# sahaRatul/sela

Hardware: NVIDIA H100
Metric: encode+decode MSamples/s (higher is better)
Workload: dtype f64+int64

## Files before the change

include/sela_b200.h:

```cpp
#ifndef SELA_B200_H_
#define SELA_B200_H_

#include <stddef.h>
#include <stdint.h>

#ifdef __cplusplus
extern "C" {
#endif

#define SELAB200_ABI_VERSION     2
#define SELAB200_FRAME_SAMPLES   2048
#define SELAB200_MAX_LPC_ORDER   100
#define SELAB200_MAX_RICE_PARAM  20
#define SELAB200_MAX_CHANNELS    16

typedef enum selab200_status {
    SELAB200_OK              = 0,
    SELAB200_ERR_NO_DEVICE   = -1,
    SELAB200_ERR_CUDA        = -2,
    SELAB200_ERR_ARGUMENT    = -3,
    SELAB200_ERR_CAPACITY    = -4,
    SELAB200_ERR_RANGE       = -5,
    SELAB200_ERR_BITSTREAM   = -6,
    SELAB200_ERR_NOT_INIT    = -7
// ... 65 lines not shown
    uint32_t header_frames;
    uint32_t n_frames;
    uint64_t n_words;
    uint64_t n_bytes_used;
} selab200_container_info;

size_t selab200_container_bound(uint32_t n_frames, uint32_t channels);

int selab200_encode_container(const int16_t *pcm, uint32_t n_frames, uint32_t channels,
                              uint32_t sample_rate, uint16_t bits_per_sample,
                              uint8_t *container, size_t capacity, size_t *bytes_used);

int selab200_container_info_get(const uint8_t *container, size_t n_bytes, selab200_container_info *info);

int selab200_container_frame_offsets(const uint8_t *container, size_t n_bytes, uint64_t *offsets,
                                     size_t capacity, selab200_container_info *info);

typedef struct selab200_container selab200_container;
int  selab200_container_open(const uint8_t *container, size_t n_bytes, selab200_container **handle,
                             selab200_container_info *info);
int  selab200_container_decode(selab200_container *handle, int16_t *pcm_out);
void selab200_container_close(selab200_container *handle);


int selab200_lpc_residues(const int32_t *samples, uint32_t n_sub, uint8_t *order,
                          int32_t *q, int32_t *residues);

int selab200_lpc_samples(const int32_t *residues, uint32_t n_sub, const uint8_t *order,
                         const int32_t *q, int32_t *samples);

int selab200_rice_encode(const int32_t *values, const uint32_t *counts, uint32_t n_streams,
                         uint32_t stride, uint32_t *rice_param, uint32_t *n_words,
                         uint32_t *words, uint32_t words_stride);

int selab200_rice_decode(const uint32_t *words, const uint32_t *n_words, uint32_t words_stride,
                         const uint32_t *rice_param, const uint32_t *counts, uint32_t n_streams,
                         int32_t *out, uint32_t out_stride);


typedef struct selab200_analysis_trace {
    double  mean;
    double  ac[101];
    double  k[100];
    int64_t c[101];
    int32_t q[100];
    int32_t order;
    int32_t reserved;
} selab200_analysis_trace;

int selab200_encode_trace(const int16_t *pcm, uint32_t n_frames, uint32_t channels,
                          selab200_subframe_desc *descs, uint32_t *words, size_t words_capacity,
                          size_t *words_used, selab200_analysis_trace *trace);

int selab200_quantise_probe(const double *k, size_t n, int32_t *out);

int selab200_fir_probe(const int32_t *samples, const int32_t *orders, const int64_t *c, uint32_t n, int wide,
                       int32_t *residues);

#ifdef __cplusplus
}
#endif
#endif
```

sela_b200/_lib.py:

```python
import ctypes as C
import pathlib

import numpy as np

PKG = pathlib.Path(__file__).resolve().parent
LIB_PATH = PKG / "libsela_b200.so"
HEADER_PATH = PKG.parent / "include" / "sela_b200.h"

FRAME = 2048
MAX_ORDER = 100

DESC_DTYPE = np.dtype([
    ("channel", "u1"), ("subframe_type", "u1"), ("parent_channel", "u1"),
    ("refl_rice_param", "u1"), ("refl_words", "<u2"), ("lpc_order", "u1"),
    ("res_rice_param", "u1"), ("res_words", "<u2"), ("samples", "<u2"),
    ("reserved", "<u4"), ("refl_offset", "<u8"), ("res_offset", "<u8"),
], align=True)
assert DESC_DTYPE.itemsize == 32

INFO_DTYPE = np.dtype([
    ("sample_rate", "<u4"), ("bits_per_sample", "<u2"), ("channels", "u1"), ("reserved", "u1"),
    ("header_frames", "<u4"), ("n_frames", "<u4"), ("n_words", "<u8"), ("n_bytes_used", "<u8"),
], align=True)
assert INFO_DTYPE.itemsize == 32

TRACE_DTYPE = np.dtype([
    ("mean", "<f8"), ("ac", "<f8", (101,)), ("k", "<f8", (100,)), ("c", "<i8", (101,)),
    ("q", "<i4", (100,)), ("order", "<i4"), ("reserved", "<i4"),
], align=True)
assert TRACE_DTYPE.itemsize == 2832

STATUS_NAMES = {0: "OK", -1: "NO_DEVICE", -2: "CUDA", -3: "ARGUMENT", -4: "CAPACITY", -5: "RANGE",
                -6: "BITSTREAM", -7: "NOT_INIT"}


class SelaB200Error(RuntimeError):
    def __init__(self, status, message):
        super().__init__("selab200 status %d (%s): %s" % (status, STATUS_NAMES.get(status, "?"), message))
        self.status = status


_lib = None

_V, _U32, _SZ, _I = C.c_void_p, C.c_uint32, C.c_size_t, C.c_int
_SIGNATURES = {
    "selab200_init": (_I, [_I]),
    "selab200_init_devices": (_I, [_I, _V]),
    "selab200_device_count": (_I, []),
    "selab200_shutdown": (None, []),
    "selab200_last_error": (C.c_char_p, []),
    "selab200_abi_version": (_I, []),
    "selab200_launch_count": (C.c_uint64, []),
    "selab200_selftest": (_I, [_V]),
    "selab200_host_alloc": (_V, [_SZ]),
    "selab200_host_free": (None, [_V]),
    "selab200_encode_words_bound": (_SZ, [_U32, _U32]),
    "selab200_encode_frames": (_I, [_V, _U32, _U32, _V, _V, _SZ, _V]),
    "selab200_decode_frames": (_I, [_V, _U32, _U32, _V, _SZ, _V]),
    "selab200_encode_workspace_bytes": (_SZ, [_U32, _U32]),
    "selab200_encode_frames_device": (_I, [_V, _U32, _U32, _V, _V, _SZ, _V, _V, _V, _SZ, _V]),
    "selab200_decode_workspace_bytes": (_SZ, [_U32, _U32]),
    "selab200_decode_frames_device": (_I, [_V, _U32, _U32, _V, _SZ, _V, _V, _V, _SZ, _V]),
    "selab200_rice_decode_frames_device": (_I, [_V, _U32, _U32, _V, _SZ, _V, _V, _V]),
    "selab200_rice_decode_flagged": (_I, [_V]),
    "selab200_container_bound": (_SZ, [_U32, _U32]),
    "selab200_encode_container": (_I, [_V, _U32, _U32, _U32, C.c_uint16, _V, _SZ, _V]),
    "selab200_container_info_get": (_I, [_V, _SZ, _V]),
    "selab200_container_frame_offsets": (_I, [_V, _SZ, _V, _SZ, _V]),
    "selab200_container_open": (_I, [_V, _SZ, _V, _V]),
    "selab200_container_decode": (_I, [_V, _V]),
    "selab200_container_close": (None, [_V]),
    "selab200_lpc_residues": (_I, [_V, _U32, _V, _V, _V]),
    "selab200_lpc_samples": (_I, [_V, _U32, _V, _V, _V]),
    "selab200_rice_encode": (_I, [_V, _V, _U32, _U32, _V, _V, _V, _U32]),
    "selab200_rice_decode": (_I, [_V, _V, _U32, _V, _V, _U32, _V, _U32]),
    "selab200_encode_trace": (_I, [_V, _U32, _U32, _V, _V, _SZ, _V, _V]),
    "selab200_quantise_probe": (_I, [_V, _SZ, _V]),
    "selab200_fir_probe": (_I, [_V, _V, _V, _U32, _I, _V]),
}


def exported_symbols():
    return sorted(_SIGNATURES)


def lib():
    global _lib
    if _lib is None:
        if not LIB_PATH.exists():
            raise ImportError("%s not built: run `python -m sela_b200.build` (nvcc, sm_90a). "
                              "There is no CPU fallback." % LIB_PATH)
        L = C.CDLL(str(LIB_PATH))
        for name, (res, args) in _SIGNATURES.items():
            fn = getattr(L, name)
            fn.restype, fn.argtypes = res, args
        _lib = L
    return _lib


def check(status):
    if status != 0:
        raise SelaB200Error(status, lib().selab200_last_error().decode(errors="replace"))


_initialised = None


def init(device=0):
    global _initialised
    key = tuple(device) if isinstance(device, (list, tuple)) else (device,)
    if _initialised != key:
        arr = (C.c_int * len(key))(*key)
        check(lib().selab200_init_devices(len(key), C.addressof(arr)))
        _initialised = key
```

sela_b200/csrc/c_abi.cu:

```cuda
#include <algorithm>
#include <atomic>
#include <cstdarg>
#include <cstdio>
#include <cstdlib>
#include <cstring>
#include <mutex>
#include <thread>
#include <vector>

#include "kernels.cuh"

using namespace selab200;

namespace {

thread_local char g_error[512] = "";
std::mutex g_mutex;
std::atomic<uint64_t> g_launches{0};

int fail(int code, const char *fmt, ...)
{
    va_list ap;
    va_start(ap, fmt);
    vsnprintf(g_error, sizeof g_error, fmt, ap);
// ... 187 lines not shown
        if (g_slots[i].ready && g_slots[i].device == attr.device) {
            tl_ctx = &g_slots[i];
            cudaError_t e = cudaSetDevice(g.device);
            if (e != cudaSuccess)
                return fail(SELAB200_ERR_CUDA, "cudaSetDevice(%d) failed: %s", g.device, cudaGetErrorString(e));
            return 0;
        }
    return fail(SELAB200_ERR_ARGUMENT, "the buffers live on device %d, which the library was not initialised for "
                                       "(selab200_init / selab200_init_devices)", attr.device);
}

size_t align256(size_t v) { return (v + 255) & ~(size_t)255; }

template <typename K>
int set_smem(K kernel, size_t bytes)
{
    static std::mutex m;
    static std::vector<std::pair<std::pair<const void *, int>, size_t>> done;
    int dev = 0;
    CUDA_TRY(cudaGetDevice(&dev));
    const std::pair<const void *, int> key(reinterpret_cast<const void *>(kernel), dev);
    std::lock_guard<std::mutex> lock(m);
    for (auto &e : done)
        if (e.first == key) {
            if (e.second >= bytes)
                return 0;
            CUDA_TRY(cudaFuncSetAttribute(kernel, cudaFuncAttributeMaxDynamicSharedMemorySize, (int)bytes));
            e.second = bytes;
            return 0;
        }
    CUDA_TRY(cudaFuncSetAttribute(kernel, cudaFuncAttributeMaxDynamicSharedMemorySize, (int)bytes));
    done.emplace_back(key, bytes);
    return 0;
}

int launch_check(const char *what)
{
    g_launches.fetch_add(1, std::memory_order_relaxed);
    cudaError_t e = cudaGetLastError();
    if (e != cudaSuccess)
        return fail(SELAB200_ERR_CUDA, "launch of %s failed: %s", what, cudaGetErrorString(e));
    return 0;
}

template <int KIND>
int launch_unit_means(const void *src, size_t n_units, uint32_t channels, double *means, cudaStream_t stream)
{
    const MeanTiling mt = mean_tiling(KIND, channels);
    k_unit_means<KIND><<<(unsigned)((n_units + 31) / 32), 32, unit_means_smem_bytes(mt), stream>>>(src, (uint32_t)n_units,
                                                                                                 channels, means);
    return launch_check("k_unit_means");
}

template <bool STEREO, bool TRACE>
int launch_encode_units(const EncodeParams &p, size_t n_units, selab200_analysis_trace *d_trace, cudaStream_t stream)
{
    constexpr size_t smem = encode_smem_bytes<STEREO>();
    if (int rc = set_smem(k_encode_units<STEREO, TRACE>, smem))
        return rc;
    k_encode_units<STEREO, TRACE><<<(unsigned)n_units, 32, smem, stream>>>(p, d_trace);
    return launch_check("k_encode_units");
}


int encode_device(const int16_t *d_pcm, uint32_t n_frames, uint32_t channels, selab200_subframe_desc *d_descs,
                  uint32_t *d_words, size_t capacity, uint64_t *d_used, int32_t *d_status, void *d_ws,
                  size_t ws_bytes, cudaStream_t stream, bool fresh = true, cudaEvent_t before_scan = nullptr,
                  cudaEvent_t after_scan = nullptr, unsigned long long *h_fill_after = nullptr,
                  uint8_t *d_container = nullptr, unsigned long long sub_base = 0,
                  selab200_analysis_trace *d_trace = nullptr)
{
    if (channels == 0 || channels > SELAB200_MAX_CHANNELS)
        return fail(SELAB200_ERR_ARGUMENT, "channels must be in [1, %d]", SELAB200_MAX_CHANNELS);
    if (ws_bytes < selab200_encode_workspace_bytes(n_frames, channels))
        return fail(SELAB200_ERR_ARGUMENT, "encode workspace too small");
    if (channels == 2 && (reinterpret_cast<uintptr_t>(d_pcm) & 15) != 0)
        return fail(SELAB200_ERR_ARGUMENT, "stereo PCM must be 16-byte aligned on the device");
    if (fresh) {
        CUDA_TRY(cudaMemsetAsync(d_status, 0, sizeof(int32_t), stream));
        CUDA_TRY(cudaMemsetAsync(d_used, 0, sizeof(uint64_t), stream));
    }
    if (n_frames == 0)
        return 0;
    const bool stereo = channels == 2;
    const size_t n_units = encode_units(n_frames, channels);
    const size_t n_sub = (size_t)n_frames * channels;
    EncodeParams p;
    p.pcm = d_pcm;
    p.n_frames = n_frames;
    p.channels = channels;
    p.descs = d_descs;
    p.words = d_words;
    p.capacity = capacity;
    p.words_used = reinterpret_cast<unsigned long long *>(d_used);
    p.status = d_status;
    p.units = static_cast<UnitRecord *>(d_ws);
    p.slots = reinterpret_cast<uint32_t *>(static_cast<char *>(d_ws) + align256(n_units * sizeof(UnitRecord)));
    p.means = reinterpret_cast<double *>(reinterpret_cast<char *>(p.slots) + align256(n_units * (size_t)kSlotWords * 4));
    p.residues = reinterpret_cast<int32_t *>(reinterpret_cast<char *>(p.means) + align256(n_units * sizeof(double)));
    if (int rc = stereo ? launch_unit_means<kMeanStereo>(d_pcm, n_units, channels, p.means, stream)
                        : launch_unit_means<kMeanPcm>(d_pcm, n_units, channels, p.means, stream))
        return rc;
    const int rc_units = stereo ? (d_trace ? launch_encode_units<true, true>(p, n_units, d_trace, stream)
                                           : launch_encode_units<true, false>(p, n_units, nullptr, stream))
                                : (d_trace ? launch_encode_units<false, true>(p, n_units, d_trace, stream)
                                           : launch_encode_units<false, false>(p, n_units, nullptr, stream));
    if (rc_units)
        return rc_units;
    const unsigned scan_ctas = (unsigned)((n_sub + kScanTile - 1) / kScanTile);
    k_encode_sizes<<<scan_ctas, kScanTile, 0, stream>>>(p);
    if (int rc = launch_check("k_encode_sizes"))
        return rc;
    if (before_scan)
        CUDA_TRY(cudaStreamWaitEvent(stream, before_scan, 0));
    k_encode_scan<<<scan_ctas, kScanTile, 0, stream>>>(p);
    if (int rc = launch_check("k_encode_scan"))
        return rc;
    CUDA_TRY(cudaMemcpyAsync(d_used, p.residues, 8, cudaMemcpyDeviceToDevice, stream));
    if (h_fill_after)
        CUDA_TRY(cudaMemcpyAsync(h_fill_after, d_used, 8, cudaMemcpyDeviceToHost, stream));
    if (after_scan)
        CUDA_TRY(cudaEventRecord(after_scan, stream));
    if (d_container) {
        k_encode_gather_container<<<(unsigned)((n_sub + 7) / 8), 256, 0, stream>>>(p, d_container, sub_base);
        return launch_check("k_encode_gather_container");
    }
    k_encode_gather<<<(unsigned)((n_sub + 7) / 8), 256, 0, stream>>>(p);
    return launch_check("k_encode_gather");
}

int launch_rice_decode(const DecodeParams &p, int which, cudaStream_t stream)
{
    const size_t n_sub = (size_t)p.n_frames * p.channels;
    const unsigned blocks = (unsigned)((n_sub + 32 * kRiceWarps - 1) / (32 * kRiceWarps));
    k_rice_decode<kRiceRing, kRiceBatch><<<blocks, 32 * kRiceWarps, 0, stream>>>(p, which);
    return launch_check(which ? "k_rice_decode(res)" : "k_rice_decode(refl)");
}

int rice_split_log2(size_t n_sub)
{
    if (const char *env = std::getenv("SELAB200_RICE_SPLIT")) {
        const long v = std::atol(env);
        if (v <= 0)
            return -1;
        int l = 0;
        while ((1 << (l + 1)) <= v && l < 4)
            l++;
        return l;
    }
    const size_t sms = (size_t)g.sms;
    if (n_sub >= 81 * sms)
        return 0;
    int l = 0;
    while (l < 4 && (n_sub << l) < 270 * sms)
        l++;
    return l;
}

template <int LOG2S>
// ... 1031 lines not shown
        return rc;
    CUDA_TRY(cudaMemcpyAsync(g.h_small + 8, d, 4, cudaMemcpyDeviceToHost, g.stream));
    CUDA_TRY(cudaStreamSynchronize(g.stream));
    *mismatches = (uint32_t)g.h_small[8];
    return 0;
}

int selab200_encode_trace(const int16_t *pcm, uint32_t n_frames, uint32_t channels, selab200_subframe_desc *descs,
                          uint32_t *words, size_t words_capacity, size_t *words_used, selab200_analysis_trace *trace)
{
    std::lock_guard<std::mutex> lock(g_mutex);
    if (int rc = require_ready())
        return rc;
    if (!pcm || !descs || !words || !words_used || !trace)
        return fail(SELAB200_ERR_ARGUMENT, "null pointer");
    if (channels == 0 || channels > SELAB200_MAX_CHANNELS)
        return fail(SELAB200_ERR_ARGUMENT, "channels must be in [1, %d]", SELAB200_MAX_CHANNELS);
    *words_used = 0;
    if (n_frames == 0)
        return 0;
    const size_t n_sub = (size_t)n_frames * channels, n_units = encode_units(n_frames, channels);
    const size_t ws_bytes = selab200_encode_workspace_bytes(n_frames, channels);
    if (int rc = g.in.ensure(n_sub * kFrame * 2)) return rc;
    if (int rc = g.descs.ensure(n_sub * sizeof(selab200_subframe_desc))) return rc;
    if (int rc = g.words.ensure(words_capacity * 4 + 64)) return rc;
    if (int rc = g.work.ensure(ws_bytes)) return rc;
    if (int rc = g.aux.ensure(n_units * sizeof(selab200_analysis_trace))) return rc;
    int32_t *d_status = static_cast<int32_t *>(g.small.ptr);
    uint64_t *d_used = reinterpret_cast<uint64_t *>(static_cast<char *>(g.small.ptr) + 8);
    selab200_analysis_trace *d_trace = static_cast<selab200_analysis_trace *>(g.aux.ptr);
    CUDA_TRY(cudaMemsetAsync(d_trace, 0, n_units * sizeof(selab200_analysis_trace), g.stream));
    CUDA_TRY(cudaMemcpyAsync(g.in.ptr, pcm, n_sub * kFrame * 2, cudaMemcpyHostToDevice, g.stream));
    if (int rc = encode_device(static_cast<const int16_t *>(g.in.ptr), n_frames, channels,
                               static_cast<selab200_subframe_desc *>(g.descs.ptr), static_cast<uint32_t *>(g.words.ptr),
                               words_capacity, d_used, d_status, g.work.ptr, g.work.bytes, g.stream, true, nullptr,
                               nullptr, nullptr, nullptr, 0, d_trace))
        return rc;
    CUDA_TRY(cudaMemcpyAsync(descs, g.descs.ptr, n_sub * sizeof(selab200_subframe_desc), cudaMemcpyDeviceToHost, g.stream));
    CUDA_TRY(cudaMemcpyAsync(trace, d_trace, n_units * sizeof(selab200_analysis_trace), cudaMemcpyDeviceToHost, g.stream));
    CUDA_TRY(cudaMemcpyAsync(g.h_small, g.small.ptr, 16, cudaMemcpyDeviceToHost, g.stream));
    CUDA_TRY(cudaStreamSynchronize(g.stream));
    uint64_t used;
    memcpy(&used, g.h_small + 2, 8);
    *words_used = (size_t)used;
    if (g.h_small[0] != 0)
        return fail(g.h_small[0], "%s", status_text(g.h_small[0]));
    if (used > words_capacity)
        return fail(SELAB200_ERR_CAPACITY, "%s", status_text(SELAB200_ERR_CAPACITY));
    CUDA_TRY(cudaMemcpyAsync(words, g.words.ptr, used * 4, cudaMemcpyDeviceToHost, g.stream));
    CUDA_TRY(cudaStreamSynchronize(g.stream));
    return 0;
}

int selab200_quantise_probe(const double *k, size_t n, int32_t *out)
{
    std::lock_guard<std::mutex> lock(g_mutex);
    if (int rc = require_ready())
        return rc;
    if (!k || !out)
        return fail(SELAB200_ERR_ARGUMENT, "null pointer");
    if (n == 0)
        return 0;
    if (n > 0xffffffffu)
        return fail(SELAB200_ERR_ARGUMENT, "at most 2^32 - 1 values per call");
    if (int rc = g.in.ensure(n * sizeof(double))) return rc;
    if (int rc = g.work.ensure(n * 4 * sizeof(int32_t))) return rc;
    CUDA_TRY(cudaMemcpyAsync(g.in.ptr, k, n * sizeof(double), cudaMemcpyHostToDevice, g.stream));
    k_quantise_probe<<<(unsigned)((n + 255) / 256), 256, 0, g.stream>>>(static_cast<const double *>(g.in.ptr), (uint32_t)n,
                                                                       static_cast<int32_t *>(g.work.ptr));
    if (int rc = launch_check("k_quantise_probe"))
        return rc;
    CUDA_TRY(cudaMemcpyAsync(out, g.work.ptr, n * 4 * sizeof(int32_t), cudaMemcpyDeviceToHost, g.stream));
    CUDA_TRY(cudaStreamSynchronize(g.stream));
    return 0;
}

int selab200_fir_probe(const int32_t *samples, const int32_t *orders, const int64_t *c, uint32_t n, int wide,
                       int32_t *residues)
{
    std::lock_guard<std::mutex> lock(g_mutex);
    if (int rc = require_ready())
        return rc;
    if (!samples || !orders || !c || !residues)
        return fail(SELAB200_ERR_ARGUMENT, "null pointer");
    if (n == 0)
        return 0;
    const int hi = wide ? 65535 : 32767, lo = wide ? -65535 : -32768;
    for (size_t i = 0; i < (size_t)n * kFrame; i++)
        if (samples[i] > hi || samples[i] < lo)
            return fail(SELAB200_ERR_RANGE, "sample %zu = %d outside the domain of the row form", i, samples[i]);
    for (uint32_t i = 0; i < n; i++)
        if (orders[i] < 0 || orders[i] > kMaxOrder)
            return fail(SELAB200_ERR_RANGE, "order %d of signal %u outside 0..%d", orders[i], i, kMaxOrder);
    const size_t sig = (size_t)n * kFrame * 4, cb = (size_t)n * (kMaxOrder + 1) * 8;
    if (int rc = g.in.ensure(sig)) return rc;
    if (int rc = g.work.ensure(sig)) return rc;
    if (int rc = g.aux.ensure(cb + (size_t)n * 4)) return rc;
    long long *d_c = static_cast<long long *>(g.aux.ptr);
    int32_t *d_orders = reinterpret_cast<int32_t *>(d_c + (size_t)n * (kMaxOrder + 1));
    CUDA_TRY(cudaMemcpyAsync(g.in.ptr, samples, sig, cudaMemcpyHostToDevice, g.stream));
    CUDA_TRY(cudaMemcpyAsync(d_c, c, cb, cudaMemcpyHostToDevice, g.stream));
    CUDA_TRY(cudaMemcpyAsync(d_orders, orders, (size_t)n * 4, cudaMemcpyHostToDevice, g.stream));
    k_fir_probe<<<n, 32, 0, g.stream>>>(static_cast<const int32_t *>(g.in.ptr), d_orders, d_c, wide,
                                        static_cast<int32_t *>(g.work.ptr));
    if (int rc = launch_check("k_fir_probe"))
        return rc;
// ... 143 lines not shown
```

sela_b200/csrc/kernels.cuh:

```cuda
#pragma once

#include "lpc.cuh"
#include "rice.cuh"
#include "rice_vs.cuh"

namespace selab200 {

enum { kMeanPcm = 0, kMeanStereo = 1, kMeanPlanar = 2 };
constexpr int kMeanTile = 64;
constexpr int kMeanSlots = 16;

struct MeanTiling {
    uint32_t units_per_row;
    uint32_t step;
    uint32_t row_stride;
    uint32_t rows_max;
    uint32_t row_words;
};

__host__ __device__ inline MeanTiling mean_tiling(int kind, uint32_t channels)
{
    MeanTiling t;
    uint32_t span = 1;
    if (kind == kMeanPcm) {
// ... 64 lines not shown
            fetch(t + 1);
#pragma unroll 8
        for (int j = 0; j < kMeanTile; j++) {
            int x;
            if (KIND == kMeanPcm) {
                x = *reinterpret_cast<const int16_t *>(at + j * mt.step);
            } else if (KIND == kMeanStereo) {
                const uint32_t pair = *reinterpret_cast<const uint32_t *>(at + 4 * j);
                const int a = (int)(pair << 16) >> 16, b = (int)pair >> 16;
                x = role == 0 ? a : role == 1 ? b : a - b;
            } else {
                x = *reinterpret_cast<const int32_t *>(at + 4 * j);
            }
            chain.add(x);
        }
    }
    if (u < n_units)
        means[u] = chain.mean();
}

inline size_t unit_means_smem_bytes(const MeanTiling &mt) { return (size_t)mt.rows_max * mt.row_words * 4; }


constexpr uint32_t kSlotWords = 1600;
constexpr uint32_t kSlotReflWords = 32;

struct __align__(16) UnitRecord {
    uint32_t order;
    uint32_t refl_k, refl_words;
    uint32_t res_k, res_words;
    uint32_t flags;
    uint32_t pad[2];
};

struct EncodeParams {
    const int16_t *pcm;
    uint32_t n_frames, channels;
    selab200_subframe_desc *descs;
    uint32_t *words;
    unsigned long long capacity;
    unsigned long long *words_used;
    int32_t *status;
    UnitRecord *units;
    uint32_t *slots;
    double *means;
    int32_t *residues;
};

__host__ __device__ inline uint32_t encode_units(uint32_t n_frames, uint32_t channels)
{
    return channels == 2 ? n_frames * 3u : n_frames * channels;
}

template <bool STEREO, bool TRACE = false>
__global__ void __launch_bounds__(32) k_encode_units(EncodeParams p, selab200_analysis_trace *trace)
{
    constexpr int kRow = kHistoryPad + kFrame;
    constexpr int kLoWords = (kHistoryPad + kFrame) / 32;
    extern __shared__ __align__(16) unsigned char smem_raw[];
    int16_t *s16 = reinterpret_cast<int16_t *>(smem_raw);
    uint32_t *lo_bits = reinterpret_cast<uint32_t *>(smem_raw + kRow * 2);
    constexpr size_t kSigBytes = kRow * 2 + (STEREO ? kLoWords * 4 : 0);
    AnalysisScratch &scratch = *reinterpret_cast<AnalysisScratch *>(smem_raw + kSigBytes);
    static_assert(kCoefAlias + sizeof(CoefSmem) <= sizeof(AnalysisScratch) && kCoefAlias % 16 == 0, "predictor alias");
    CoefSmem &cf = *reinterpret_cast<CoefSmem *>(smem_raw + kSigBytes + kCoefAlias);

    const int lane = lane_id();
    const uint32_t unit = blockIdx.x;
    const uint32_t frame = STEREO ? unit / 3 : unit / p.channels;
    const uint32_t role = STEREO ? unit % 3 : unit % p.channels;

    const int16_t *src = p.pcm + (size_t)frame * kFrame * p.channels;
    for (int j = lane; j < kHistoryPad / 2; j += 32)
        reinterpret_cast<uint32_t *>(s16)[j] = 0;
    int16_t *row = s16 + kHistoryPad;
    Signal sig;
    sig.a = row;
    sig.lo = nullptr;
    if (STEREO) {
        const uint4 *src128 = reinterpret_cast<const uint4 *>(src);
        if (role < 2) {
            const uint32_t sel = role ? 0x7632 : 0x5410;
            for (int j = lane; j < kFrame / 4; j += 32) {
                const uint4 v = src128[j];
                reinterpret_cast<uint2 *>(row)[j] = make_uint2(__byte_perm(v.x, v.y, sel), __byte_perm(v.z, v.w, sel));
            }
        } else {
            if (lane < kHistoryPad / 32)
                lo_bits[lane] = 0;
            uint32_t *lo = lo_bits + kHistoryPad / 32;
            for (int it = 0; it < kFrame / 128; it++) {
                const uint4 v = src128[it * 32 + lane];
                const uint32_t pr[4] = {v.x, v.y, v.z, v.w};
                int d[4];
#pragma unroll
                for (int e = 0; e < 4; e++)
                    d[e] = ((int)(pr[e] << 16) >> 16) - ((int)pr[e] >> 16);
                const uint32_t h01 = ((uint32_t)(d[0] >> 1) & 0xffffu) | ((uint32_t)(d[1] >> 1) << 16);
                const uint32_t h23 = ((uint32_t)(d[2] >> 1) & 0xffffu) | ((uint32_t)(d[3] >> 1) << 16);
                reinterpret_cast<uint2 *>(row)[it * 32 + lane] = make_uint2(h01, h23);
                uint32_t nib = (d[0] & 1) | ((d[1] & 1) << 1) | ((d[2] & 1) << 2) | ((d[3] & 1) << 3);
                nib <<= 4 * (lane & 7);
                nib |= __shfl_xor_sync(kFull, nib, 1);
                nib |= __shfl_xor_sync(kFull, nib, 2);
                nib |= __shfl_xor_sync(kFull, nib, 4);
                if ((lane & 7) == 0)
                    lo[it * 4 + (lane >> 3)] = nib;
            }
            sig.lo = lo;
        }
    } else {
        for (int j = lane; j < kFrame; j += 32)
            row[j] = src[(size_t)j * p.channels + role];
    }
    __syncwarp();

    int32_t *res = p.residues + (size_t)unit * kFrame;
    warp_autocorrelation(sig, scratch, shfl_d(lane == 0 ? p.means[unit] : 0.0, 0));
    if constexpr (TRACE) {
        selab200_analysis_trace &tr = trace[unit];
        if (lane == 0)
            tr.mean = p.means[unit];
        for (int i = lane; i <= kMaxOrder; i += 32)
            tr.ac[i] = scratch.ac[i];
    }
    warp_schur(scratch);
    const int order = warp_order_and_quantise(scratch, cf);
    warp_coefficients(cf, scratch.t(), order);
    if constexpr (TRACE) {
        selab200_analysis_trace &tr = trace[unit];
        for (int i = lane; i < kMaxOrder; i += 32) {
            tr.k[i] = scratch.kk()[i];
            tr.q[i] = cf.q[i];
        }
        for (int i = lane; i <= kMaxOrder; i += 32)
            tr.c[i] = i == 0 ? 0 : coef_at(cf, i);
        if (lane == 0)
            tr.order = order;
    }
    static_assert(kPlaneBytes <= kCoefAlias, "FIR digit planes");
    uint32_t *planes = reinterpret_cast<uint32_t *>(scratch.ring);
    if (STEREO && role == 2)
        warp_fir_residual<true>(sig, cf, order, planes, res);
    else
        warp_fir_residual<false>(sig, cf, order, planes, res);

    const RiceChoice cq = warp_rice_choose(cf.q, order);
    const RiceChoice cr = warp_rice_choose(res, kFrame);
    const bool too_large = cq.words > kSlotReflWords || cr.words > kSlotWords - kSlotReflWords;
    uint32_t *slot = p.slots + (size_t)unit * kSlotWords;
    if (!too_large) {
        warp_rice_pack(cf.q, order, cq, slot);
        warp_rice_pack(res, kFrame, cr, slot + kSlotReflWords);
    }
    __syncwarp();
    for (int l = lane; l < kFrame * 4 / 128; l += 32)
        asm volatile("discard.global.L2 [%0], 128;" ::"l"(res + l * 32) : "memory");
    if (lane == 0) {
        UnitRecord u;
        u.order = order;
        u.refl_k = cq.k;
        u.refl_words = cq.words;
        u.res_k = cr.k;
        u.res_words = cr.words;
        u.flags = too_large ? 1u : 0u;
        u.pad[0] = u.pad[1] = 0;
        p.units[unit] = u;
    }
}

template <bool STEREO>
constexpr size_t encode_smem_bytes()
{
    return (size_t)(kHistoryPad + kFrame) * 2 + (STEREO ? (kHistoryPad + kFrame) / 8 : 0) + sizeof(AnalysisScratch);
}

__device__ __forceinline__ void warp_copy_words(uint32_t *__restrict__ dst, const uint32_t *__restrict__ src, uint32_t n, int lane)
{
    for (uint32_t w = lane; w < n; w += 256) {
        uint32_t v[8];
#pragma unroll
        for (int j = 0; j < 8; j++)
            v[j] = w + 32 * j < n ? __ldcs(src + w + 32 * j) : 0u;
#pragma unroll
        for (int j = 0; j < 8; j++)
            if (w + 32 * j < n)
                dst[w + 32 * j] = v[j];
    }
}

struct Emit {
    uint32_t unit, type, parent;
};
__device__ __forceinline__ Emit choose_unit(const UnitRecord *units, uint32_t channels, uint32_t sub)
{
    Emit e;
    if (channels != 2) {
        e.unit = sub;
        e.type = 0;
        e.parent = sub % channels;
        return e;
    }
    const uint32_t frame = sub >> 1;
    if ((sub & 1) == 0) {
        e.unit = 3 * frame;
        e.type = 0;
        e.parent = 0;
        return e;
    }
    const UnitRecord a = units[3 * frame + 1], d = units[3 * frame + 2];
    const bool diff_wins = (unsigned long long)d.refl_words + d.res_words <
                           (unsigned long long)a.refl_words + a.res_words;
    e.unit = 3 * frame + (diff_wins ? 2 : 1);
    e.type = diff_wins ? 1 : 0;
    e.parent = diff_wins ? 0 : 1;
    return e;
}

__device__ __forceinline__ Emit choose_record(const UnitRecord *units, uint32_t channels, uint32_t sub, UnitRecord &u)
{
// ... 642 lines not shown
__global__ void __launch_bounds__(128) k_diff_fixup(DecodeParams p)
{
    const uint32_t frame = blockIdx.x;
    const selab200_subframe_desc *fd = p.descs + (size_t)frame * 2;
    const selab200_subframe_desc d0 = fd[0], d1 = fd[1];
    if (!desc_ok(d0, 2, p.n_words) || !desc_ok(d1, 2, p.n_words) || d0.channel == d1.channel)
        return;
    if ((d0.subframe_type | d1.subframe_type) == 0 || (d0.subframe_type & d1.subframe_type))
        return;
    const uint32_t pos = d1.subframe_type ? 1 : 0;
    const selab200_subframe_desc d = pos ? d1 : d0;
    const int32_t *diff = p.ws_res + ((size_t)frame * 2 + pos) * kFrame;
    int16_t *out = p.pcm_out + (size_t)frame * kFrame * 2;
    for (int t = threadIdx.x; t < kFrame; t += blockDim.x)
        out[2 * t + d.channel] = (int16_t)(uint16_t)((int)out[2 * t + d.parent_channel] - diff[t]);
}

inline size_t synthesise_smem_bytes(uint32_t ch)
{
    return (size_t)ch * kFrame * 4 + ch * (sizeof(CoefSmem) + sizeof(IirSmem)) +
           ((ch + 1) / 2) * 104 * sizeof(double) + (2 * ch + 1) * sizeof(int);
}


struct Row17 {
    __align__(16) int16_t a[kHistoryPad + kFrame];
    uint32_t lo[(kHistoryPad + kFrame) / 32];
    __device__ __forceinline__ Signal stage(const int32_t *src)
    {
        const int lane = lane_id();
        for (int i = lane; i < kHistoryPad / 2; i += 32)
            reinterpret_cast<uint32_t *>(a)[i] = 0;
        if (lane < kHistoryPad / 32)
            lo[lane] = 0;
        stage_17bit_row(src, a + kHistoryPad, lo + kHistoryPad / 32);
        __syncwarp();
        return Signal{a + kHistoryPad, lo + kHistoryPad / 32};
    }
};

__global__ void __launch_bounds__(32) k_lpc_residues(const int32_t *samples, const double *means, uint32_t n_sub,
                                                     uint8_t *order_out, int32_t *q_out, int32_t *residues)
{
    __shared__ __align__(16) AnalysisScratch scratch;
    __shared__ __align__(16) CoefSmem cf;
    __shared__ __align__(16) Row17 row;
    const uint32_t sub = blockIdx.x;
    const int lane = lane_id();
    const Signal sig = row.stage(samples + (size_t)sub * kFrame);
    warp_autocorrelation(sig, scratch, means[sub]);
    warp_schur(scratch);
    const int order = warp_order_and_quantise(scratch, cf);
    warp_coefficients(cf, scratch.t(), order);
    warp_fir_residual<true>(sig, cf, order, reinterpret_cast<uint32_t *>(scratch.ring), residues + (size_t)sub * kFrame);
    for (int i = lane; i < kMaxOrder; i += 32)
        q_out[(size_t)sub * kMaxOrder + i] = i < order ? cf.q[i] : 0;
    if (lane == 0)
        order_out[sub] = (uint8_t)order;
}

__global__ void __launch_bounds__(32) k_fir_probe(const int32_t *samples, const int32_t *orders, const long long *c,
                                                  int wide, int32_t *residues)
{
    __shared__ __align__(16) AnalysisScratch scratch;
    __shared__ __align__(16) CoefSmem cf;
    __shared__ __align__(16) Row17 row;
    const uint32_t sub = blockIdx.x;
    const int lane = lane_id();
    const int32_t *src = samples + (size_t)sub * kFrame;
    Signal sig = row.stage(src);
    if (!wide) {
        for (int j = lane; j < kFrame; j += 32)
            row.a[kHistoryPad + j] = (int16_t)src[j];
        sig.lo = nullptr;
    }
    const int order = orders[sub];
    for (int i = lane; i < 112; i += 32) {
        const long long v = i < order ? c[(size_t)sub * (kMaxOrder + 1) + i + 1] : 0;
        cf.clo[i] = (uint32_t)v;
        cf.chi[i] = (int32_t)(v >> 32);
    }
    __syncwarp();
    uint32_t *planes = reinterpret_cast<uint32_t *>(scratch.ring);
    int32_t *res = residues + (size_t)sub * kFrame;
    if (wide)
        warp_fir_residual<true>(sig, cf, order, planes, res);
    else
        warp_fir_residual<false>(sig, cf, order, planes, res);
}

__global__ void __launch_bounds__(32) k_lpc_samples(const int32_t *residues, uint32_t n_sub, const uint8_t *order_in,
                                                    const int32_t *q_in, int32_t *samples)
{
    __shared__ __align__(16) CoefSmem cf;
    __shared__ __align__(16) IirSmem ii;
    __shared__ double t[104];
    __shared__ __align__(16) int32_t buf[kFrame];
    const uint32_t sub = blockIdx.x;
    const int lane = lane_id();
    int order = order_in[sub];
    if (order > kMaxOrder)
        order = kMaxOrder;
    for (int i = lane; i < 104; i += 32)
        cf.q[i] = i < order ? q_in[(size_t)sub * kMaxOrder + i] : 0;
    for (int i = lane; i < kFrame; i += 32)
        buf[i] = residues[(size_t)sub * kFrame + i];
    __syncwarp();
    warp_coefficients(cf, t, order);
    warp_iir_prepare(cf, ii, order);
    warp_iir_synthesis_pair(cf, ii, order, buf, lane < 16, kFrame);
    for (int i = lane; i < kFrame; i += 32)
        samples[(size_t)sub * kFrame + i] = buf[i];
}

__global__ void k_quantise_probe(const double *k, uint32_t n, int32_t *out)
{
    const uint32_t i = blockIdx.x * blockDim.x + threadIdx.x;
    if (i >= n)
        return;
    const double kv = k[i];
    out[4 * (size_t)i + 0] = quantise_reflection(0, kv);
    out[4 * (size_t)i + 1] = quantise_reflection(1, kv);
    out[4 * (size_t)i + 2] = quantise_reflection(2, kv);
    out[4 * (size_t)i + 3] = reflection_significant(kv) ? 1 : 0;
}

__global__ void k_selftest_scaling(uint32_t *mismatches)
{
    const int s = (int)(blockIdx.x * blockDim.x + threadIdx.x) - 65535;
    if (s > 65535)
        return;
    if (__double_as_longlong(sample_to_x(s)) != __double_as_longlong(sample_to_x_div(s)))
        atomicAdd(mismatches, 1u);
}

__global__ void __launch_bounds__(32) k_rice_encode(const int32_t *values, const uint32_t *counts, uint32_t pitch,
// ... 47 lines not shown
```

sela_b200/csrc/lpc.cuh:

```cuda
#pragma once

#include "common.cuh"
#include "lpc_tables.cuh"

namespace selab200 {

struct CoefSmem {
    uint32_t clo[112];
    int32_t  chi[112];
    int32_t  q[104];
};
struct IirSmem {
    unsigned long long pre[104];
};
struct AnalysisScratch {
    double ring[256];
    double ac[128];
    __device__ __forceinline__ double *kk() { return ring; }
    __device__ __forceinline__ double *t() { return ring + 104; }
};
using LpcSmem = AnalysisScratch;
constexpr size_t kCoefAlias = 208 * sizeof(double);

__device__ __forceinline__ long long coef_at(const CoefSmem &cf, int j)
// ... 189 lines not shown
    return order;
}

__device__ __forceinline__ double dequantise(int i, int q)
{
    int idx = q + 64;
    idx = idx < 0 ? 0 : (idx > 127 ? 127 : idx);
    if (i == 0)
        return __longlong_as_double((long long)selab200_FIRST_BITS[idx]);
    if (i == 1)
        return idx == 0 ? __longlong_as_double((long long)SELAB200_SECOND0_BITS)
                        : -__longlong_as_double((long long)selab200_FIRST_BITS[idx]);
    return (double)(idx - 64) / 64.0;
}

__device__ void warp_coefficients(CoefSmem &cf, double *t, int order)
{
    const int lane = lane_id();
    for (int i = lane; i < 112; i += 32) {
        cf.clo[i] = 0;
        cf.chi[i] = 0;
    }
    __syncwarp();
    if (order <= 1)
        return;
    for (int i = 0; i < order; i++) {
        const double ki = dequantise(i, cf.q[i]);
        const int half = i >> 1;
        for (int j = lane; j < half; j += 32) {
            double a = t[j];
            double b = t[i - 1 - j];
            t[j] = dadd(a, dmul(ki, b));
            t[i - 1 - j] = dadd(b, dmul(ki, a));
        }
        if (lane == 0) {
            if (i & 1) {
                double mid = t[half];
                t[half] = dadd(mid, dmul(mid, ki));
            }
            t[i] = ki;
        }
        __syncwarp();
    }
    const double scale = 34359738368.0;
    for (int m = lane; m < order; m += 32) {
        const long long v = __double2ll_rz(dmul(scale, -t[m]));
        cf.clo[m] = (uint32_t)v;
        cf.chi[m] = (int32_t)(v >> 32);
    }
    __syncwarp();
}

constexpr int kPlaneWords = 34;
constexpr size_t kPlaneBytes = 8 * kPlaneWords * 4;

__device__ int warp_fir_planes(const CoefSmem &cf, uint32_t *planes)
{
    const unsigned long long H = 0x8080808080808080ull;
    const int lane = lane_id();
    __syncwarp();
    int nd = 0;
    for (int w = lane; w < kPlaneWords; w += 32) {
        unsigned long long e[4];
#pragma unroll
        for (int i = 0; i < 4; i++) {
            const int j = 4 * w + i - 7;
            const unsigned long long c = (j >= 1 && j <= 112) ? (unsigned long long)coef_at(cf, j) : 0ull;
            e[i] = (c + H) ^ H;
            nd = max(nd, (64 - __clzll((long long)e[i]) + 7) >> 3);
        }
#pragma unroll
        for (int p = 0; p < 8; p++) {
            uint32_t v = 0;
#pragma unroll
            for (int i = 0; i < 4; i++)
                v |= (uint32_t)((e[i] >> (8 * p)) & 0xffu) << (8 * i);
            planes[p * kPlaneWords + w] = v;
        }
    }
    __syncwarp();
    return __reduce_max_sync(kFull, nd);
}

__device__ __forceinline__ uint32_t prmt(uint32_t x, uint32_t y, uint32_t sel)
{
    uint32_t d;
    asm("prmt.b32 %0, %1, %2, %3;" : "=r"(d) : "r"(x), "r"(y), "r"(sel));
    return d;
}

template <bool ASIGNED>
__device__ __forceinline__ void mma_s8(int32_t (&d)[4], const uint32_t (&a)[4], uint32_t b0, uint32_t b1)
{
    if constexpr (ASIGNED)
        asm("mma.sync.aligned.m16n8k32.row.col.s32.s8.s8.s32 {%0,%1,%2,%3}, {%4,%5,%6,%7}, {%8,%9}, {%0,%1,%2,%3};"
            : "+r"(d[0]), "+r"(d[1]), "+r"(d[2]), "+r"(d[3])
            : "r"(a[0]), "r"(a[1]), "r"(a[2]), "r"(a[3]), "r"(b0), "r"(b1));
    else
        asm("mma.sync.aligned.m16n8k32.row.col.s32.u8.s8.s32 {%0,%1,%2,%3}, {%4,%5,%6,%7}, {%8,%9}, {%0,%1,%2,%3};"
            : "+r"(d[0]), "+r"(d[1]), "+r"(d[2]), "+r"(d[3])
            : "r"(a[0]), "r"(a[1]), "r"(a[2]), "r"(a[3]), "r"(b0), "r"(b1));
}

__device__ __forceinline__ unsigned long long mad_wide_s32(int32_t a, int32_t b, unsigned long long c)
{
    unsigned long long d;
    asm("mad.wide.s32 %0, %1, %2, %3;" : "=l"(d) : "r"(a), "r"(b), "l"(c));
    return d;
}

template <bool WIDE>
__device__ void warp_fir_residual(const Signal &sig, const CoefSmem &cf, int order, uint32_t *planes, int32_t *res)
{
    constexpr int NL = WIDE ? 3 : 2;
    const int lane = lane_id();
    const int g = lane >> 2, t = lane & 3;
    const int nd = warp_fir_planes(cf, planes);
    const int ksteps = (order + 8 + 31) >> 5;
    const uint32_t *pg = planes + t + (g >> 2);
    const uint32_t sh = 8 * (g & 3);
    for (int mt = 0; mt < kFrame / 128; mt++) {
        int32_t T[8][4];
#pragma unroll
        for (int k = 0; k < 8; k++)
            T[k][0] = T[k][1] = T[k][2] = T[k][3] = 0;
        for (int ks = 0; ks < ksteps; ks++) {
            const int s0 = 128 * mt + 8 * g + 4 - 4 * t - 32 * ks;
            constexpr int kOff[4] = {0, 64, -16, 48};
            uint32_t A[NL][4];
#pragma unroll
            for (int r = 0; r < 4; r++) {
                const int j = s0 + kOff[r];
                const uint2 v = *reinterpret_cast<const uint2 *>(sig.a + j);
                if constexpr (WIDE) {
                    const uint32_t x = v.x << 1, y = v.y << 1;
                    const uint32_t nib = (sig.lo[j >> 5] >> (j & 31)) & 0xfu;
                    const uint32_t par = ((nib * 0x08040201u) >> 3) & 0x01010101u;
                    A[0][r] = (prmt(x, y, 0x0246) & 0xfefefefeu) | par;
                    A[1][r] = prmt(x, y, 0x1357);
                    A[2][r] = prmt(v.x, v.y, 0x9bdf);
                } else {
                    A[0][r] = prmt(v.x, v.y, 0x0246);
                    A[1][r] = prmt(v.x, v.y, 0x1357);
                }
            }
            const uint32_t *pk = pg + 8 * ks;
#pragma unroll
            for (int p = 0; p < 8; p++) {
                if (p < nd) {
                    const uint32_t *w = pk + p * kPlaneWords;
                    const uint32_t b0 = __funnelshift_r(w[0], w[1], sh);
                    const uint32_t b1 = __funnelshift_r(w[4], w[5], sh);
                    mma_s8<false>(T[p], A[0], b0, b1);
                    if (p + 1 < 8)
                        mma_s8<!WIDE>(T[p + 1], A[1], b0, b1);
                    if constexpr (WIDE)
                        if (p + 2 < 8)
                            mma_s8<true>(T[p + 2], A[2], b0, b1);
                }
            }
        }
        const int i0 = 128 * mt + 8 * g + 2 * t;
#pragma unroll
        for (int h = 0; h < 2; h++) {
            const int i = i0 + 64 * h;
            const uint32_t pair = *reinterpret_cast<const uint32_t *>(sig.a + i);
            int s[2] = {(int)(pair << 16) >> 16, (int)pair >> 16};
            if constexpr (WIDE) {
                const uint32_t bits = sig.lo[i >> 5] >> (i & 31);
                s[0] = 2 * s[0] + (int)(bits & 1u);
                s[1] = 2 * s[1] + (int)((bits >> 1) & 1u);
            }
            int32_t out[2];
#pragma unroll
            for (int e = 0; e < 2; e++) {
                const int r = 2 * h + e;
                unsigned long long sum = 1ull << (kQ - 1);
#pragma unroll
                for (int k = 0; k < 4; k++)
                    sum = mad_wide_s32(T[k][r], 1 << (8 * k), sum);
                const uint32_t top = (uint32_t)T[4][r] + ((uint32_t)T[5][r] << 8) + ((uint32_t)T[6][r] << 16) +
                                     ((uint32_t)T[7][r] << 24);
                sum += (unsigned long long)top << 32;
                out[e] = s[e] - (int32_t)((long long)sum >> kQ);
            }
            *reinterpret_cast<int2 *>(res + i) = make_int2(out[0], out[1]);
        }
    }
    __syncwarp();
}

__device__ void warp_iir_prepare(const CoefSmem &cf, IirSmem &ii, int order)
{
    const int lane = lane_id();
    long long v[4], run = 0;
#pragma unroll
    for (int m = 0; m < 4; m++) {
        const int j = 4 * lane + m + 1;
        run += (j <= order && j <= 112) ? coef_at(cf, j) : 0;
        v[m] = run;
    }
    unsigned long long incl = (unsigned long long)run;
#pragma unroll
    for (int o = 1; o < 32; o <<= 1) {
        unsigned long long tmp = __shfl_up_sync(kFull, incl, o);
        if (lane >= o)
            incl += tmp;
    }
    const unsigned long long excl = incl - (unsigned long long)run;
#pragma unroll
    for (int m = 0; m < 4; m++) {
        const int j = 4 * lane + m + 1;
        if (j < 104)
            ii.pre[j] = (1ull << (kQ - 1)) + ((excl + (unsigned long long)v[m]) << 31);
    }
    if (lane == 0)
        ii.pre[0] = 1ull << (kQ - 1);
    __syncwarp();
}

template <int TPL>
__device__ void warp_iir_pair(const CoefSmem &cf, const IirSmem &ii, int order, int32_t *buf, bool active, int n, int order_max)
{
    const int hl = lane_id() & 15;
    uint32_t cl[TPL];
    int32_t ch[TPL];
#pragma unroll
    for (int m = 0; m < TPL; m++) {
        const int j = TPL * hl + m;
        cl[m] = j < 112 ? cf.clo[j] : 0u;
        ch[m] = j < 112 ? cf.chi[j] : 0;
    }
    unsigned long long alo[TPL];
    uint32_t ahi[TPL];
#pragma unroll
    for (int m = 0; m < TPL; m++) {
        alo[m] = 0;
        ahi[m] = 0;
    }
    const unsigned long long steady = ii.pre[order];
    uint32_t sp = synth_biased(buf[0]);
// ... 190 lines not shown
```

Measured before the change: 11170.

## Pre-pair FIR digit planes as uint2 and specialise tile loop on digit count

Each FIR digit-plane word is now stored together with its next neighbour as a uint2, built with warp shuffles. The MMA loop can then fetch both funnel-shift operands in one 64-bit shared load. The tile loop is templated on the number of digit planes (5 or 8), so the per-plane runtime branch goes away and fully unrolled code is emitted for each case. The MMA issue order is reversed. A separate CLOCKS instrumentation path records per-phase clock64 timestamps, but it only runs through a new probe entry point. The cost is doubled plane storage in shared memory and extra code size.

```diff
diff --git a/include/sela_b200.h b/include/sela_b200.h
--- a/include/sela_b200.h
+++ b/include/sela_b200.h
@@ -141,6 +141,9 @@
                           selab200_subframe_desc *descs, uint32_t *words, size_t words_capacity,
                           size_t *words_used, selab200_analysis_trace *trace);
 
+#define SELAB200_ENCODE_CLOCK_SLOTS 9
+int selab200_encode_phase_clocks(const int16_t *pcm, uint32_t n_frames, uint32_t channels, uint64_t *clocks);
+
 int selab200_quantise_probe(const double *k, size_t n, int32_t *out);
 
 int selab200_fir_probe(const int32_t *samples, const int32_t *orders, const int64_t *c, uint32_t n, int wide,
diff --git a/sela_b200/_lib.py b/sela_b200/_lib.py
--- a/sela_b200/_lib.py
+++ b/sela_b200/_lib.py
@@ -75,6 +75,7 @@
     "selab200_rice_encode": (_I, [_V, _V, _U32, _U32, _V, _V, _V, _U32]),
     "selab200_rice_decode": (_I, [_V, _V, _U32, _V, _V, _U32, _V, _U32]),
     "selab200_encode_trace": (_I, [_V, _U32, _U32, _V, _V, _SZ, _V, _V]),
+    "selab200_encode_phase_clocks": (_I, [_V, _U32, _U32, _V]),
     "selab200_quantise_probe": (_I, [_V, _SZ, _V]),
     "selab200_fir_probe": (_I, [_V, _V, _V, _U32, _I, _V]),
 }
diff --git a/sela_b200/csrc/c_abi.cu b/sela_b200/csrc/c_abi.cu
--- a/sela_b200/csrc/c_abi.cu
+++ b/sela_b200/csrc/c_abi.cu
@@ -263,13 +263,14 @@
     return launch_check("k_unit_means");
 }
 
-template <bool STEREO, bool TRACE>
-int launch_encode_units(const EncodeParams &p, size_t n_units, selab200_analysis_trace *d_trace, cudaStream_t stream)
+template <bool STEREO, bool TRACE, bool CLOCKS = false>
+int launch_encode_units(const EncodeParams &p, size_t n_units, selab200_analysis_trace *d_trace, cudaStream_t stream,
+                        unsigned long long *d_clocks = nullptr)
 {
     constexpr size_t smem = encode_smem_bytes<STEREO>();
-    if (int rc = set_smem(k_encode_units<STEREO, TRACE>, smem))
-        return rc;
-    k_encode_units<STEREO, TRACE><<<(unsigned)n_units, 32, smem, stream>>>(p, d_trace);
+    if (int rc = set_smem(k_encode_units<STEREO, TRACE, CLOCKS>, smem))
+        return rc;
+    k_encode_units<STEREO, TRACE, CLOCKS><<<(unsigned)n_units, 32, smem, stream>>>(p, d_trace, d_clocks);
     return launch_check("k_encode_units");
 }
 
@@ -279,7 +280,7 @@
                   size_t ws_bytes, cudaStream_t stream, bool fresh = true, cudaEvent_t before_scan = nullptr,
                   cudaEvent_t after_scan = nullptr, unsigned long long *h_fill_after = nullptr,
                   uint8_t *d_container = nullptr, unsigned long long sub_base = 0,
-                  selab200_analysis_trace *d_trace = nullptr)
+                  selab200_analysis_trace *d_trace = nullptr, unsigned long long *d_clocks = nullptr)
 {
     if (channels == 0 || channels > SELAB200_MAX_CHANNELS)
         return fail(SELAB200_ERR_ARGUMENT, "channels must be in [1, %d]", SELAB200_MAX_CHANNELS);
@@ -312,10 +313,15 @@
     if (int rc = stereo ? launch_unit_means<kMeanStereo>(d_pcm, n_units, channels, p.means, stream)
                         : launch_unit_means<kMeanPcm>(d_pcm, n_units, channels, p.means, stream))
         return rc;
-    const int rc_units = stereo ? (d_trace ? launch_encode_units<true, true>(p, n_units, d_trace, stream)
-                                           : launch_encode_units<true, false>(p, n_units, nullptr, stream))
-                                : (d_trace ? launch_encode_units<false, true>(p, n_units, d_trace, stream)
-                                           : launch_encode_units<false, false>(p, n_units, nullptr, stream));
+    int rc_units;
+    if (d_clocks)
+        rc_units = stereo ? launch_encode_units<true, false, true>(p, n_units, nullptr, stream, d_clocks)
+                          : launch_encode_units<false, false, true>(p, n_units, nullptr, stream, d_clocks);
+    else
+        rc_units = stereo ? (d_trace ? launch_encode_units<true, true>(p, n_units, d_trace, stream)
+                                     : launch_encode_units<true, false>(p, n_units, nullptr, stream))
+                          : (d_trace ? launch_encode_units<false, true>(p, n_units, d_trace, stream)
+                                     : launch_encode_units<false, false>(p, n_units, nullptr, stream));
     if (rc_units)
         return rc_units;
     const unsigned scan_ctas = (unsigned)((n_sub + kScanTile - 1) / kScanTile);
@@ -1453,6 +1459,43 @@
     return 0;
 }
 
+int selab200_encode_phase_clocks(const int16_t *pcm, uint32_t n_frames, uint32_t channels, uint64_t *clocks)
+{
+    std::lock_guard<std::mutex> lock(g_mutex);
+    if (int rc = require_ready())
+        return rc;
+    if (!pcm || !clocks)
+        return fail(SELAB200_ERR_ARGUMENT, "null pointer");
+    if (channels == 0 || channels > SELAB200_MAX_CHANNELS)
+        return fail(SELAB200_ERR_ARGUMENT, "channels must be in [1, %d]", SELAB200_MAX_CHANNELS);
+    if (n_frames == 0)
+        return 0;
+    const size_t n_sub = (size_t)n_frames * channels, n_units = encode_units(n_frames, channels);
+    const size_t ws_bytes = selab200_encode_workspace_bytes(n_frames, channels);
+    const size_t capacity = selab200_encode_words_bound(n_frames, channels);
+    const size_t clock_bytes = n_units * SELAB200_ENCODE_CLOCK_SLOTS * sizeof(uint64_t);
+    if (int rc = g.in.ensure(n_sub * kFrame * 2)) return rc;
+    if (int rc = g.descs.ensure(n_sub * sizeof(selab200_subframe_desc))) return rc;
+    if (int rc = g.words.ensure(capacity * 4 + 64)) return rc;
+    if (int rc = g.work.ensure(ws_bytes)) return rc;
+    if (int rc = g.aux.ensure(clock_bytes)) return rc;
+    int32_t *d_status = static_cast<int32_t *>(g.small.ptr);
+    uint64_t *d_used = reinterpret_cast<uint64_t *>(static_cast<char *>(g.small.ptr) + 8);
+    unsigned long long *d_clocks = static_cast<unsigned long long *>(g.aux.ptr);
+    CUDA_TRY(cudaMemcpyAsync(g.in.ptr, pcm, n_sub * kFrame * 2, cudaMemcpyHostToDevice, g.stream));
+    if (int rc = encode_device(static_cast<const int16_t *>(g.in.ptr), n_frames, channels,
+                               static_cast<selab200_subframe_desc *>(g.descs.ptr), static_cast<uint32_t *>(g.words.ptr),
+                               capacity, d_used, d_status, g.work.ptr, g.work.bytes, g.stream, true, nullptr, nullptr,
+                               nullptr, nullptr, 0, nullptr, d_clocks))
+        return rc;
+    CUDA_TRY(cudaMemcpyAsync(clocks, d_clocks, clock_bytes, cudaMemcpyDeviceToHost, g.stream));
+    CUDA_TRY(cudaMemcpyAsync(g.h_small, g.small.ptr, 4, cudaMemcpyDeviceToHost, g.stream));
+    CUDA_TRY(cudaStreamSynchronize(g.stream));
+    if (g.h_small[0] != 0)
+        return fail(g.h_small[0], "%s", status_text(g.h_small[0]));
+    return 0;
+}
+
 int selab200_quantise_probe(const double *k, size_t n, int32_t *out)
 {
     std::lock_guard<std::mutex> lock(g_mutex);
diff --git a/sela_b200/csrc/kernels.cuh b/sela_b200/csrc/kernels.cuh
--- a/sela_b200/csrc/kernels.cuh
+++ b/sela_b200/csrc/kernels.cuh
@@ -140,9 +140,11 @@
     return channels == 2 ? n_frames * 3u : n_frames * channels;
 }
 
-template <bool STEREO, bool TRACE = false>
-__global__ void __launch_bounds__(32) k_encode_units(EncodeParams p, selab200_analysis_trace *trace)
-{
+template <bool STEREO, bool TRACE = false, bool CLOCKS = false>
+__global__ void __launch_bounds__(32) k_encode_units(EncodeParams p, selab200_analysis_trace *trace,
+                                                 unsigned long long *clocks)
+{
+    static_assert(!(TRACE && CLOCKS), "the trace's copies would be timed with the phases");
     constexpr int kRow = kHistoryPad + kFrame;
     constexpr int kLoWords = (kHistoryPad + kFrame) / 32;
     extern __shared__ __align__(16) unsigned char smem_raw[];
@@ -157,6 +159,14 @@
     const uint32_t unit = blockIdx.x;
     const uint32_t frame = STEREO ? unit / 3 : unit / p.channels;
     const uint32_t role = STEREO ? unit % 3 : unit % p.channels;
+    const auto mark = [&](int i) {
+        if constexpr (CLOCKS) {
+            __syncwarp();
+            if (lane == 0)
+                clocks[(size_t)unit * SELAB200_ENCODE_CLOCK_SLOTS + i] = clock64();
+        }
+    };
+    mark(0);
 
     const int16_t *src = p.pcm + (size_t)frame * kFrame * p.channels;
     for (int j = lane; j < kHistoryPad / 2; j += 32)
@@ -202,9 +212,11 @@
             row[j] = src[(size_t)j * p.channels + role];
     }
     __syncwarp();
+    mark(1);
 
     int32_t *res = p.residues + (size_t)unit * kFrame;
     warp_autocorrelation(sig, scratch, shfl_d(lane == 0 ? p.means[unit] : 0.0, 0));
+    mark(2);
     if constexpr (TRACE) {
         selab200_analysis_trace &tr = trace[unit];
         if (lane == 0)
@@ -213,8 +225,10 @@
             tr.ac[i] = scratch.ac[i];
     }
     warp_schur(scratch);
+    mark(3);
     const int order = warp_order_and_quantise(scratch, cf);
     warp_coefficients(cf, scratch.t(), order);
+    mark(4);
     if constexpr (TRACE) {
         selab200_analysis_trace &tr = trace[unit];
         for (int i = lane; i < kMaxOrder; i += 32) {
@@ -226,15 +240,17 @@
         if (lane == 0)
             tr.order = order;
     }
-    static_assert(kPlaneBytes <= kCoefAlias, "FIR digit planes");
-    uint32_t *planes = reinterpret_cast<uint32_t *>(scratch.ring);
+    static_assert(kPlaneBytes <= kCoefAlias + offsetof(CoefSmem, q), "FIR digit planes");
+    uint2 *planes = reinterpret_cast<uint2 *>(scratch.ring);
     if (STEREO && role == 2)
         warp_fir_residual<true>(sig, cf, order, planes, res);
     else
         warp_fir_residual<false>(sig, cf, order, planes, res);
+    mark(5);
 
     const RiceChoice cq = warp_rice_choose(cf.q, order);
     const RiceChoice cr = warp_rice_choose(res, kFrame);
+    mark(6);
     const bool too_large = cq.words > kSlotReflWords || cr.words > kSlotWords - kSlotReflWords;
     uint32_t *slot = p.slots + (size_t)unit * kSlotWords;
     if (!too_large) {
@@ -254,6 +270,14 @@
         u.flags = too_large ? 1u : 0u;
         u.pad[0] = u.pad[1] = 0;
         p.units[unit] = u;
+    }
+    mark(7);
+    if constexpr (CLOCKS) {
+        if (lane == 0) {
+            uint32_t sm;
+            asm volatile("mov.u32 %0, %%smid;" : "=r"(sm));
+            clocks[(size_t)unit * SELAB200_ENCODE_CLOCK_SLOTS + 8] = sm;
+        }
     }
 }
 
@@ -1002,7 +1026,8 @@
     warp_schur(scratch);
     const int order = warp_order_and_quantise(scratch, cf);
     warp_coefficients(cf, scratch.t(), order);
-    warp_fir_residual<true>(sig, cf, order, reinterpret_cast<uint32_t *>(scratch.ring), residues + (size_t)sub * kFrame);
+    static_assert(kPlaneBytes <= sizeof(AnalysisScratch), "FIR digit planes");
+    warp_fir_residual<true>(sig, cf, order, reinterpret_cast<uint2 *>(scratch.ring), residues + (size_t)sub * kFrame);
     for (int i = lane; i < kMaxOrder; i += 32)
         q_out[(size_t)sub * kMaxOrder + i] = i < order ? cf.q[i] : 0;
     if (lane == 0)
@@ -1031,7 +1056,7 @@
         cf.chi[i] = (int32_t)(v >> 32);
     }
     __syncwarp();
-    uint32_t *planes = reinterpret_cast<uint32_t *>(scratch.ring);
+    uint2 *planes = reinterpret_cast<uint2 *>(scratch.ring);
     int32_t *res = residues + (size_t)sub * kFrame;
     if (wide)
         warp_fir_residual<true>(sig, cf, order, planes, res);
diff --git a/sela_b200/csrc/lpc.cuh b/sela_b200/csrc/lpc.cuh
--- a/sela_b200/csrc/lpc.cuh
+++ b/sela_b200/csrc/lpc.cuh
@@ -265,15 +265,18 @@
 }
 
 constexpr int kPlaneWords = 34;
-constexpr size_t kPlaneBytes = 8 * kPlaneWords * 4;
-
-__device__ int warp_fir_planes(const CoefSmem &cf, uint32_t *planes)
+constexpr size_t kPlaneBytes = 8 * kPlaneWords * sizeof(uint2);
+
+__device__ int warp_fir_planes(const CoefSmem &cf, uint2 *planes)
 {
     const unsigned long long H = 0x8080808080808080ull;
     const int lane = lane_id();
     __syncwarp();
     int nd = 0;
-    for (int w = lane; w < kPlaneWords; w += 32) {
+    uint32_t v[2][8];
+#pragma unroll
+    for (int h = 0; h < 2; h++) {
+        const int w = lane + 32 * h;
         unsigned long long e[4];
 #pragma unroll
         for (int i = 0; i < 4; i++) {
@@ -284,12 +287,21 @@
         }
 #pragma unroll
         for (int p = 0; p < 8; p++) {
-            uint32_t v = 0;
+            uint32_t x = 0;
 #pragma unroll
             for (int i = 0; i < 4; i++)
-                v |= (uint32_t)((e[i] >> (8 * p)) & 0xffu) << (8 * i);
-            planes[p * kPlaneWords + w] = v;
-        }
+                x |= (uint32_t)((e[i] >> (8 * p)) & 0xffu) << (8 * i);
+            v[h][p] = x;
+        }
+    }
+    __syncwarp();
+#pragma unroll
+    for (int p = 0; p < 8; p++) {
+        const uint32_t n0 = __shfl_sync(kFull, v[0][p], (lane + 1) & 31);
+        const uint32_t n1 = __shfl_sync(kFull, v[1][p], (lane + 1) & 31);
+        planes[p * kPlaneWords + lane] = make_uint2(v[0][p], lane < 31 ? n0 : n1);
+        if (lane + 32 < kPlaneWords)
+            planes[p * kPlaneWords + lane + 32] = make_uint2(v[1][p], n1);
     }
     __syncwarp();
     return __reduce_max_sync(kFull, nd);
@@ -322,15 +334,13 @@
     return d;
 }
 
-template <bool WIDE>
-__device__ void warp_fir_residual(const Signal &sig, const CoefSmem &cf, int order, uint32_t *planes, int32_t *res)
+template <bool WIDE, int ND>
+__device__ __forceinline__ void warp_fir_tiles(const Signal &sig, int ksteps, const uint2 *planes, int32_t *res)
 {
     constexpr int NL = WIDE ? 3 : 2;
     const int lane = lane_id();
     const int g = lane >> 2, t = lane & 3;
-    const int nd = warp_fir_planes(cf, planes);
-    const int ksteps = (order + 8 + 31) >> 5;
-    const uint32_t *pg = planes + t + (g >> 2);
+    const uint2 *pg = planes + t + (g >> 2);
     const uint32_t sh = 8 * (g & 3);
     for (int mt = 0; mt < kFrame / 128; mt++) {
         int32_t T[8][4];
@@ -357,20 +367,18 @@
                     A[1][r] = prmt(v.x, v.y, 0x1357);
                 }
             }
-            const uint32_t *pk = pg + 8 * ks;
-#pragma unroll
-            for (int p = 0; p < 8; p++) {
-                if (p < nd) {
-                    const uint32_t *w = pk + p * kPlaneWords;
-                    const uint32_t b0 = __funnelshift_r(w[0], w[1], sh);
-                    const uint32_t b1 = __funnelshift_r(w[4], w[5], sh);
-                    mma_s8<false>(T[p], A[0], b0, b1);
-                    if (p + 1 < 8)
-                        mma_s8<!WIDE>(T[p + 1], A[1], b0, b1);
-                    if constexpr (WIDE)
-                        if (p + 2 < 8)
-                            mma_s8<true>(T[p + 2], A[2], b0, b1);
-                }
+            const uint2 *pk = pg + 8 * ks;
+#pragma unroll
+            for (int p = 0; p < ND; p++) {
+                const uint2 lo = pk[p * kPlaneWords], hi = pk[p * kPlaneWords + 4];
+                const uint32_t b0 = __funnelshift_r(lo.x, lo.y, sh);
+                const uint32_t b1 = __funnelshift_r(hi.x, hi.y, sh);
+                if constexpr (WIDE)
+                    if (p + 2 < 8)
+                        mma_s8<true>(T[p + 2], A[2], b0, b1);
+                if (p + 1 < 8)
+                    mma_s8<!WIDE>(T[p + 1], A[1], b0, b1);
+                mma_s8<false>(T[p], A[0], b0, b1);
             }
         }
         const int i0 = 128 * mt + 8 * g + 2 * t;
@@ -400,6 +408,17 @@
             *reinterpret_cast<int2 *>(res + i) = make_int2(out[0], out[1]);
         }
     }
+}
+
+template <bool WIDE>
+__device__ void warp_fir_residual(const Signal &sig, const CoefSmem &cf, int order, uint2 *planes, int32_t *res)
+{
+    const int nd = warp_fir_planes(cf, planes);
+    const int ksteps = (order + 8 + 31) >> 5;
+    if (nd <= 5)
+        warp_fir_tiles<WIDE, 5>(sig, ksteps, planes, res);
+    else
+        warp_fir_tiles<WIDE, 8>(sig, ksteps, planes, res);
     __syncwarp();
 }
 
```

Result: faster. 11380, median of 6 (+1.9%).
